# mikostrzewa/AprilSLAM

Hardware: AMD Instinct MI355X
Metric: frames/sec at 1280x720, 20 tags/frame (detection + batched PnP) (higher is better)
Workload: dtype u8/f64

## Files before the change

### aprilslam_amd/csrc/aprilslam.hip

```cpp
#include "../../include/aprilslam.h"

#include <algorithm>
#include <chrono>
#include <cmath>
#include <cstdarg>
#include <cstdio>
#include <cstring>
#include <memory>
#include <string>
#include <type_traits>
#include <vector>

#include "asl_common.h"
#include "tag_standard41h12.inc"
#include "k_wave.inc"

#include "k_threshold.inc"
#include "k_cc.inc"
#include "k_cluster.inc"
#include "k_seg.inc"
#include "k_quad.inc"
#include "k_decode.inc"
#include "k_pnp.inc"
#include "k_dedup.inc"
// ... 231 lines not shown

extern "C" int asl_detector_set_pnp_both_minima(asl_detector *d, int enabled)
{
    if (!d) return fail(ASL_EINVAL, "detector is NULL");
    d->pnp_both_minima = enabled ? 1 : 0;
    return ASL_OK;
}

extern "C" int asl_set_profiling(asl_detector *d, int enabled)
{
    if (!d) return fail(ASL_EINVAL, "detector is NULL");
    d->profiling = enabled ? 1 : 0;
    if (enabled)
        for (int i = 0; i <= MAX_STAGES; i++)
            if (!d->ev[i]) HIPCHK(hipEventCreate(&d->ev[i]));
    return ASL_OK;
}

extern "C" int asl_stage_times(asl_detector *d, const char **names, float *ms, int max_n, int *n)
{
    if (!d || !n) return fail(ASL_EINVAL, "NULL argument");
    int k = std::min(max_n, d->nstages);
    for (int i = 0; i < k; i++) { if (names) names[i] = d->stage_names[i]; if (ms) ms[i] = d->stage_ms[i]; }
    static const char *hn[4] = {"host_enqueue", "host_wait", "host_copy", "host_post"};
    for (int i = 0; i < 4 && k < max_n; i++, k++) { if (names) names[k] = hn[i]; if (ms) ms[k] = d->host_ms[i]; }
    *n = k;
    return ASL_OK;
}

static int pnp_tpw(size_t expected)
{
    const char *e = getenv("ASL_PNP_TPW");
    if (e) { int x = atoi(e); return x < 1 ? 1 : (x > 16 ? 16 : x); }
    int v = 1;
    while (v < 16 && (size_t)v * 2 * 1024 <= expected) v <<= 1;
    return v;
}

static unsigned int next_pow2(unsigned long long v)
{
    unsigned long long p = 1;
    while (p < v) p <<= 1;
    return (unsigned int)p;
}

static int make_geom(asl_detector *d, int n_frames, int channels, int w, int h, int stride, size_t frame_pitch, Geom *g)
{
    if (n_frames <= 0 || n_frames > 65535) return fail(ASL_EINVAL, "n_frames must be in [1, 65535] (got %d)", n_frames);
    if (channels != 1 && channels != 3) return fail(ASL_EINVAL, "channels must be 1 (gray) or 3 (BGR), got %d", channels);
    if (w < 8 || h < 8 || w > 16384 || h > 16384) return fail(ASL_EINVAL, "unsupported image size %dx%d", w, h);
    if (stride < w * channels) return fail(ASL_EINVAL, "stride %d smaller than a row (%d bytes)", stride, w * channels);
    g->w = w; g->h = h; g->stride = stride; g->channels = channels; g->f = d->decimate;
    g->sw = 1 + (w - 1) / g->f; g->sh = 1 + (h - 1) / g->f;
    g->tw = g->sw / TILESZ; g->th = g->sh / TILESZ;
    g->nframes = n_frames; g->frame_pitch = frame_pitch;
    g->npix = (size_t)g->sw * g->sh;
    if (g->npix >= (1u << 24)) return fail(ASL_EINVAL, "decimated frame has %zu pixels; the cluster key holds 2^24", g->npix);
    return ASL_OK;
}

static int seg_nwx(const Geom &g) { return (g.sw + 63) / 64; }
static int seg_point_tiles_y(const Geom &g) { return std::max(1, (g.sh - 1 + SEG_PH - 1) / SEG_PH); }
static size_t count_tiles(const Geom &g) { return (size_t)seg_nwx(g) * (size_t)seg_point_tiles_y(g); }

static int ensure_workspace(asl_detector *d, const Geom &g)
{
    size_t B = (size_t)g.nframes;
    size_t total = B * g.npix;
    d->nslots = next_pow2(std::max<unsigned long long>(16384ull, (unsigned long long)B * d->hash_slots_per_frame));
    unsigned long long mc = (unsigned long long)B * d->clusters_per_frame;
    d->max_clusters = (unsigned int)std::min<unsigned long long>(mc, 0x7FFFFFFFull);
    unsigned long long mp = (unsigned long long)((double)total * d->points_per_pixel) + 65536ull;
    d->max_points = (unsigned int)std::min<unsigned long long>(mp, 0xFFFFFFF0ull);
    d->max_dets = (unsigned int)std::min<unsigned long long>((unsigned long long)B * d->dets_per_frame, 0x7FFFFFFFull);
    int bad = 0;
    bad |= d->dgray.ensure(total);
    bad |= d->tmin.ensure(B * (size_t)std::max(1, g.tw * g.th) + 8);
    bad |= d->tmax.ensure(B * (size_t)std::max(1, g.tw * g.th) + 8);
    bad |= d->tcut.ensure(B * (size_t)std::max(1, g.tw * g.th));
    bad |= d->parent.ensure(total);
    bad |= d->sizes.ensure(total);
    bad |= d->rootmask.ensure(B * (size_t)g.sh * (size_t)seg_nwx(g));
    bad |= d->wmask.ensure(B * (size_t)g.sh * (size_t)seg_nwx(g));
    bad |= d->bmask.ensure(B * (size_t)g.sh * (size_t)seg_nwx(g));
    bad |= d->hkeys.ensure(d->nslots);
    bad |= d->hcounts.ensure(d->nslots);
    bad |= d->class_lists.ensure((size_t)NCLASSES * d->max_clusters);
    bad |= d->slot_cluster.ensure(d->nslots);
    bad |= d->clusters.ensure(d->max_clusters);
    bad |= d->quads.ensure(d->max_clusters);
    bad |= d->quad_list.ensure(d->max_clusters);
    bad |= d->quadH.ensure((size_t)10 * d->max_clusters);
    bad |= d->side_mom.ensure((size_t)24 * d->max_clusters);
    bad |= d->points.ensure(d->max_points);
    d->stage_cap = (unsigned int)((double)g.npix * d->points_per_pixel) + 1024u;
    bad |= d->stage_rec.ensure((size_t)B * d->stage_cap);
    bad |= d->stage_pos.ensure((size_t)B * d->stage_cap);
    bad |= d->frame_cursor.ensure(B);
    bad |= d->dense_tiles.ensure(B * count_tiles(g));
    bad |= d->dense_seg.ensure(B * (size_t)seg_nwx(g) * (size_t)((g.sh + SEG_TH - 1) / SEG_TH));
    bad |= d->seg_edges.ensure(B * (size_t)seg_nwx(g) * (size_t)((g.sh + SEG_TH - 1) / SEG_TH));
    bad |= d->scratch.ensure((size_t)d->max_points * 8);
    bad |= d->dets.ensure(d->max_dets);
    bad |= d->frame_ndets.ensure(B);
    bad |= d->frame_nkeep.ensure(B);
    bad |= d->frame_off.ensure(B);
    bad |= d->frame_idx.ensure(B * (size_t)d->dets_per_frame);
    bad |= d->out_det.ensure(d->max_dets);
    bad |= d->out_pose.ensure(d->max_dets);
    bad |= d->counters.ensure(CNT__N);
    if (bad) return fail(ASL_ENOMEM, "device workspace allocation failed (%zu frames of %dx%d)", B, g.sw, g.sh);
    return ASL_OK;
}

#define STAGE(name)                                                        \
    do {                                                                   \
        if (d->profiling && d->nev < MAX_STAGES) {                         \
            d->stage_names[d->nev] = name;                                 \
            HIPCHK(hipEventRecord(d->ev[d->nev], st));                     \
            d->nev++;                                                      \
        }                                                                  \
    } while (0)

static int tag_width(const asl_detector *d, const Geom &g) { return std::max(3, d->fam.width_at_border / g.f); }

template <int BLOCK, int CAP>
static void launch_fit(asl_detector *d, const Geom &g, int cls, unsigned int grid, hipStream_t st)
{
    const int want_rev = d->fam.reversed_border ? 1 : 0, want_norm = d->fam.reversed_border ? 0 : 1;
    hipLaunchKernelGGL((k_fit_quads<BLOCK, (CAP > 0), CAP / BLOCK>), dim3(grid), dim3(BLOCK), CAP > 0 ? QUAD_LDS_BYTES(CAP) : 0, st, d->clusters.p,
                       d->class_lists.p + (size_t)cls * d->max_clusters, d->counters.p, cls, d->max_clusters, CAP, d->points.p, d->dgray.p, g,
                       tag_width(d, g), want_rev, want_norm, d->scratch.p, d->quads.p, d->wtab.p, d->side_mom.p);
}

static void launch_fit_class(asl_detector *d, const Geom &g, int cls, unsigned int B, hipStream_t st)
{
    const unsigned int qgrid = std::min<unsigned int>(d->max_clusters, std::max<unsigned int>(16384u, 32u * B));
    const unsigned int q2grid = std::min<unsigned int>(d->max_clusters, 2048u);
    switch (cls) {
    case 0: return launch_fit<64, CLASS0_CAP>(d, g, 0, qgrid, st);
    case 1: return launch_fit<128, CLASS1_CAP>(d, g, 1, qgrid, st);
    case 2: return launch_fit<256, CLASS2_CAP>(d, g, 2, q2grid, st);
    case 3: return launch_fit<256, CLASS3_CAP>(d, g, 3, q2grid, st);
    default: return launch_fit<256, 0>(d, g, 4, q2grid, st);
    }
}

static void launch_quad_finish(asl_detector *d, const Geom &g, hipStream_t st)
{
    hipLaunchKernelGGL(k_quad_finish, dim3(std::min<unsigned int>((d->max_clusters + 63) / 64, 4096u)), dim3(256), 0, st, d->quads.p, d->side_mom.p, d->counters.p,
                       d->max_clusters, tag_width(d, g));
}

static int enqueue_detect(asl_detector *d, const uint8_t *d_frames, const Geom &g, hipStream_t st, const CamDev *cam)
{
    dim3 blk(64, 4, 1);
    int thx = (g.sh + TILESZ - 1) / TILESZ;
    unsigned int B = (unsigned int)g.nframes;
    d->nev = 0;
    range_push("S0-S4 gray, decimate, threshold, segmentation, clusters");
    STAGE("k_hash_clear");
    hipLaunchKernelGGL(k_hash_clear, dim3((std::max<unsigned int>(d->nslots, std::max<unsigned int>(B, CNT__N)) + 255) / 256), dim3(256), 0, st, d->hkeys.p,
                       d->hcounts.p, d->nslots, d->counters.p, d->frame_cursor.p, d->frame_ndets.p, B);

    STAGE("k_decimate_minmax");
    if (g.f == 2) {
        const unsigned int ntile = (unsigned int)(g.tw * g.th);
        const unsigned int nrest = (unsigned int)(g.sw - 4 * g.tw) * (unsigned int)g.sh + (unsigned int)(g.sh - 4 * g.th) * (unsigned int)(4 * g.tw);
        if (ntile)
            hipLaunchKernelGGL((g.channels == 1 ? k_decimate2_tiles<1> : k_decimate2_tiles<3>), dim3((ntile + 255) / 256, B), dim3(256), 0, st, d_frames, g,
                               d->dgray.p, d->tmin.p, d->tmax.p);
        if (nrest)
            hipLaunchKernelGGL((g.channels == 1 ? k_decimate_rest<1> : k_decimate_rest<3>), dim3((nrest + 255) / 256, B), dim3(256), 0, st, d_frames, g,
                               d->dgray.p);
    } else
        hipLaunchKernelGGL((g.channels == 1 ? k_decimate_minmax<1> : k_decimate_minmax<3>), dim3((g.sw + 63) / 64, (thx + 3) / 4, B), blk, 0, st, d_frames, g, d->dgray.p, d->tmin.p, d->tmax.p);

    const int nwx = seg_nwx(g), pty = seg_point_tiles_y(g);
    const size_t nwords = (size_t)B * g.sh * nwx;
    STAGE("k_tile_cut");
    if (g.tw > 0 && g.th > 0)
        hipLaunchKernelGGL(k_tile_cut, dim3((((g.tw + 3) / 4) * ((g.th + 3) / 4) + 255) / 256, B), dim3(256), 0, st, d->tmin.p, d->tmax.p, g, d->tcut.p);
    STAGE("k_seg_tile");
    {
        const int ntiles = nwx * ((g.sh + SEG_TH - 1) / SEG_TH);
        hipLaunchKernelGGL(k_seg_tile, dim3((ntiles + SEG_TILE_WAVES - 1) / SEG_TILE_WAVES, 1, B), dim3(64 * SEG_TILE_WAVES), 0, st, d->dgray.p, d->tcut.p, g, nwx, ntiles,
                           d->wmask.p, d->bmask.p, d->parent.p, d->sizes.p, d->rootmask.p, d->seg_edges.p, d->dense_seg.p, d->counters.p);
        hipLaunchKernelGGL(k_seg_tile_dense, dim3(1024), dim3(64), 0, st, g, nwx, ntiles, d->wmask.p, d->bmask.p, d->parent.p, d->sizes.p,
                           d->rootmask.p, d->dense_seg.p, d->counters.p);
    }
    STAGE("k_seg_border");
    {
        const size_t nseams = nwx > 1 ? (size_t)B * g.sh * (nwx - 1) : 0;
        const unsigned int ncol_blocks = (unsigned int)((nseams + 63) / 64);
        const int nrb = (g.sh - 1) / SEG_TH;
        const unsigned int nrow_blocks = (unsigned int)nwx * (unsigned int)nrb * (unsigned int)B;
        if (ncol_blocks + nrow_blocks > 0)
            hipLaunchKernelGGL(k_seg_border, dim3(ncol_blocks + nrow_blocks), dim3(64), 0, st, d->wmask.p, d->bmask.p, d->seg_edges.p,
                               nwx * ((g.sh + SEG_TH - 1) / SEG_TH), g, nwx, d->parent.p, d->counters.p, ncol_blocks, nrb > 0 ? nrb : 1);
    }
    STAGE("k_seg_roots");
    hipLaunchKernelGGL(k_seg_roots, dim3((unsigned int)((nwords + 255) / 256)), dim3(256), 0, st, d->rootmask.p, g, nwx, d->parent.p, d->sizes.p);

    STAGE("k_seg_points");
    hipLaunchKernelGGL((k_seg_points<SEGP_PCAP, SEGP_RUNCAP, SEGP_NW, 1>), dim3(B, (nwx + SEGP_NW - 1) / SEGP_NW, pty), dim3(64 * SEGP_NW), 0, st,
                       d->wmask.p, d->bmask.p, g, nwx, d->parent.p, d->sizes.p, d->hkeys.p, d->hcounts.p, d->nslots - 1, d->stage_rec.p,
                       d->stage_pos.p, d->frame_cursor.p, d->stage_cap, d->dense_tiles.p, pty, d->counters.p);
    hipLaunchKernelGGL((k_seg_points<SEGP_PCAP_DENSE, SEGP_RUNCAP_DENSE, 1, 2>), dim3(256), dim3(64), 0, st, d->wmask.p, d->bmask.p, g, nwx,
                       d->parent.p, d->sizes.p, d->hkeys.p, d->hcounts.p, d->nslots - 1, d->stage_rec.p, d->stage_pos.p, d->frame_cursor.p,
                       d->stage_cap, d->dense_tiles.p, pty, d->counters.p);
    STAGE("k_cluster_filter");
    hipLaunchKernelGGL(k_cluster_filter, dim3((d->nslots + 1023) / 1024), dim3(1024), 0, st, d->hkeys.p, d->hcounts.p, d->nslots, g,
                       d->clusters.p, d->slot_cluster.p, d->class_lists.p, d->max_clusters, d->max_points, d->counters.p);
    STAGE("k_point_place");
    hipLaunchKernelGGL(k_point_place, dim3(16, B), dim3(256), 0, st, d->stage_rec.p, d->stage_pos.p, d->frame_cursor.p, d->stage_cap,
                       d->slot_cluster.p, d->points.p, d->counters.p);

    range_pop();
    range_push("S5 quad fit");
    for (int cls = 0; cls < NCLASSES; cls++) {
        static const char *const kFitStage[NCLASSES] = {"k_fit_quads<0>", "k_fit_quads<1>", "k_fit_quads<2>", "k_fit_quads<3>", "k_fit_quads<4>"};
        STAGE(kFitStage[cls]);
        launch_fit_class(d, g, cls, B, st);
    }

    STAGE("k_quad_finish");
    launch_quad_finish(d, g, st);
    range_pop();
    range_push("S6-S7 edge refinement, homography, decode");
    STAGE("k_quad_compact");
    hipLaunchKernelGGL(k_quad_compact, dim3((d->max_clusters + 1023) / 1024), dim3(1024), 0, st, d->quads.p, d->counters.p, d->max_clusters,
                       d->quad_list.p);
    unsigned int dgrid = std::min<unsigned int>(d->max_clusters, std::max<unsigned int>(8192u, 64u * B));
    STAGE("k_refine");
    hipLaunchKernelGGL((g.channels == 1 ? k_refine<1> : k_refine<3>), dim3(dgrid), dim3(64), 0, st, d->quads.p, d->counters.p, d->max_clusters, d_frames, g,
                       d->fam.reversed_border ? 1 : 0, d->refine, d->quadH.p, d->quad_list.p, d->side_mom.p);
    STAGE("k_homography");
    hipLaunchKernelGGL(k_homography, dim3(std::min<unsigned int>((d->max_clusters + 31) / 32, 2048u)), dim3(256), 0, st, d->quadH.p, d->counters.p, d->max_clusters,
                       d->quad_list.p, d->side_mom.p);
    STAGE("k_decode");
    hipLaunchKernelGGL((g.channels == 1 ? k_decode<1> : k_decode<3>), dim3(dgrid), dim3(64), 0, st, d->quads.p, d->quadH.p, d->counters.p, d->max_clusters, d_frames, g, d->fam,
                       d->maxhamming, d->dets.p, d->max_dets, d->counters.p, d->quad_list.p);

    range_pop();
    range_push("S9 PnP, S8 de-duplication");
    if (cam) {
        STAGE("k_pnp_dets");
        const int tpw = pnp_tpw(d->nd_guess ? d->nd_guess : (size_t)20 * B);
        hipLaunchKernelGGL(k_pnp_dets, dim3((d->max_dets + tpw - 1) / tpw), dim3(64), 0, st, d->dets.p, d->counters.p, d->max_dets, *cam, tpw);
    }
    STAGE("k_det_dedup");
    {
        const unsigned int cap_f = d->dets_per_frame;
        hipLaunchKernelGGL(k_det_bucket, dim3((d->max_dets + 255) / 256), dim3(256), 0, st, d->dets.p, d->counters.p, d->max_dets, d->frame_ndets.p,
                           d->frame_idx.p, cap_f, d->counters.p);
        hipLaunchKernelGGL(k_det_dedup, dim3(B), dim3(256), 0, st, d->dets.p, d->counters.p, d->frame_ndets.p, d->frame_idx.p, cap_f,
                           d->frame_nkeep.p, d->counters.p);
        hipLaunchKernelGGL(k_det_offsets, dim3(1), dim3(1024), 0, st, d->frame_nkeep.p, B, d->frame_off.p, d->counters.p);
        hipLaunchKernelGGL(k_det_gather, dim3((cap_f + 255) / 256, B), dim3(256), 0, st, d->dets.p, d->frame_idx.p, cap_f, d->frame_nkeep.p,
                           d->frame_off.p, d->out_det.p, d->out_pose.p, d->max_dets, cam ? 1 : 0);
    }
    range_pop();
    if (d->profiling && d->nev <= MAX_STAGES) HIPCHK(hipEventRecord(d->ev[d->nev], st));
    HIPCHK(hipGetLastError());
    return ASL_OK;
}

static CamDev make_cam(const asl_detector *d, const double *K, const double *dist, int n_dist, double tag_size)
{
    CamDev c;
    c.both_minima = d->pnp_both_minima; c.pad = 0;
    c.fx = K[0]; c.fy = K[4]; c.cx = K[2]; c.cy = K[5];
    c.k1 = c.k2 = c.p1 = c.p2 = c.k3 = 0;
    if (dist && n_dist >= 4) { c.k1 = dist[0]; c.k2 = dist[1]; c.p1 = dist[2]; c.p2 = dist[3]; }
    if (dist && n_dist >= 5) c.k3 = dist[4];
    c.half = (double)(float)(tag_size / 2);
    return c;
}

using clk = std::chrono::steady_clock;
static float msf(clk::time_point a, clk::time_point b) { return std::chrono::duration<float, std::milli>(b - a).count(); }

static int ensure_host_out(asl_detector *d, size_t want, size_t nframes)
{
    HIPCHK(d->host_nkeep.ensure(nframes, hipHostMallocDefault));
    if (want <= d->host_cap()) return ASL_OK;
    d->host_det.release(); d->host_pose.release();
    want = std::max<size_t>(want * 2, 4096);
    HIPCHK(d->host_det.ensure(want, hipHostMallocNonCoherent));
    HIPCHK(d->host_pose.ensure(want, hipHostMallocNonCoherent));
    return ASL_OK;
}

static int submit_batch(asl_detector *d, const uint8_t *d_frames, const Geom &g, hipStream_t st, const CamDev *cam)
{
    if (d->pending) return fail(ASL_EINVAL, "a batch is already in flight on this detector: collect it first");
    int rc = ensure_workspace(d, g);
    if (rc) return rc;
    d->t_submit = clk::now();
    rc = enqueue_detect(d, d_frames, g, st, cam);
    if (rc) return rc;
    HIPCHK(d->pinned_counters.ensure(CNT__N, hipHostMallocDefault));
    HIPCHK(hipMemcpyAsync(d->pinned_counters.p, d->counters.p, sizeof(long long) * CNT__N, hipMemcpyDeviceToHost, st));
    d->prefetched = 0;
    rc = ensure_host_out(d, std::min<size_t>(d->nd_guess, d->max_dets), (size_t)g.nframes);
    if (rc) return rc;
    HIPCHK(hipMemcpyAsync(d->host_nkeep.p, d->frame_nkeep.p, sizeof(unsigned int) * (size_t)g.nframes, hipMemcpyDeviceToHost, st));
    if (d->nd_guess > 0) {
        size_t guess = std::min<size_t>(d->nd_guess, d->max_dets);
        HIPCHK(hipMemcpyAsync(d->host_det.p, d->out_det.p, guess * sizeof(DetOut), hipMemcpyDeviceToHost, st));
        if (cam) HIPCHK(hipMemcpyAsync(d->host_pose.p, d->out_pose.p, guess * sizeof(PoseOut), hipMemcpyDeviceToHost, st));
        d->prefetched = guess;
    }
    d->pending = true;
    d->p_frames = d_frames; d->p_geom = g; d->p_stream = st; d->p_has_cam = cam != nullptr;
    if (cam) d->p_cam = *cam;
    d->t_enqueued = clk::now();
    return ASL_OK;
}

static int collect_batch(asl_detector *d, asl_detection *out, asl_pose *poses, int max_out, int *n_per_frame, int *n_out)
{
    if (!d->pending) return fail(ASL_EINVAL, "no batch in flight on this detector");
    const Geom g = d->p_geom;
    hipStream_t st = d->p_stream;
    const CamDev *cam = d->p_has_cam ? &d->p_cam : nullptr;
    clk::time_point t0 = d->t_submit, t1 = d->t_enqueued, t2 = t1;
    for (int attempt = 0; attempt < 4; attempt++) {
        if (attempt > 0) {
            d->pending = false;
            d->nd_guess = 0;
            int rc = submit_batch(d, d->p_frames, g, st, cam);
            if (rc) return rc;
        }
        HIPCHK(hipStreamSynchronize(st));
        t2 = clk::now();
        memcpy(d->last_counters, d->pinned_counters.p, sizeof(long long) * CNT__N);
        d->last = g;
        long long *c = d->last_counters;
        if (c[CNT_UF_GUARD]) {
            d->pending = false;
            return fail(ASL_ECAPACITY, "a union-find loop hit its iteration guard (%lld times): labels of this batch are not trustworthy", c[CNT_UF_GUARD]);
        }
        bool again = false;
        if (c[CNT_OVERFLOW_HASH]) { d->hash_slots_per_frame *= 4; again = true; }
        if (c[CNT_OVERFLOW_CLUSTERS] || c[CNT_NCLUSTERS] > (long long)d->max_clusters) { d->clusters_per_frame *= 4; again = true; }
        if (c[CNT_OVERFLOW_POINTS]) { d->points_per_pixel *= 2; again = true; }
        if (c[CNT_OVERFLOW_DETS]) { d->dets_per_frame *= 4; again = true; }
        if (again) {
            if (attempt == 3) {
                d->pending = false;
                return fail(ASL_ECAPACITY, "work buffers still overflow after growing (hash %lld clusters %lld points %lld dets %lld)",
                            c[CNT_OVERFLOW_HASH], c[CNT_OVERFLOW_CLUSTERS], c[CNT_OVERFLOW_POINTS], c[CNT_OVERFLOW_DETS]);
            }
            continue;
        }
        break;
    }
    d->pending = false;
    if (d->profiling) {
        d->nstages = d->nev;
        for (int i = 0; i < d->nev; i++) HIPCHK(hipEventElapsedTime(&d->stage_ms[i], d->ev[i], d->ev[i + 1]));
    }
    if (d->last_counters[CNT_DEDUP_LIMIT])
        return fail(ASL_ECAPACITY, "%lld frame(s) hold more than %d detections: the de-duplication does not sort that many", d->last_counters[CNT_DEDUP_LIMIT], DEDUP_MAX);
    size_t nd = (size_t)d->last_counters[CNT_NKEEP];
    if (nd > d->max_dets) nd = d->max_dets;
    if (nd > d->prefetched) {
        size_t have = d->prefetched;
        if (nd > d->host_cap()) have = 0;
        int rc = ensure_host_out(d, nd, (size_t)g.nframes);
        if (rc) return rc;
        HIPCHK(hipMemcpy(d->host_det.p + have, d->out_det.p + have, (nd - have) * sizeof(DetOut), hipMemcpyDeviceToHost));
        if (cam) HIPCHK(hipMemcpy(d->host_pose.p + have, d->out_pose.p + have, (nd - have) * sizeof(PoseOut), hipMemcpyDeviceToHost));
    }
    d->nd_guess = nd + nd / 4 + 256;
    clk::time_point t3 = clk::now();
    static_assert(sizeof(DetOut) == sizeof(asl_detection) && sizeof(PoseOut) == sizeof(asl_pose), "device results are copied verbatim");
    int total = (int)nd;
    int nw = std::min(total, max_out);
    if (out && nw > 0) memcpy(out, d->host_det.p, (size_t)nw * sizeof(asl_detection));
    if (poses && cam && nw > 0) memcpy(poses, d->host_pose.p, (size_t)nw * sizeof(asl_pose));
    if (n_per_frame) for (int f = 0; f < g.nframes; f++) n_per_frame[f] = (int)d->host_nkeep.p[f];
    if (n_out) *n_out = total;
    d->host_ms[0] = msf(t0, t1); d->host_ms[1] = msf(t1, t2); d->host_ms[2] = msf(t2, t3); d->host_ms[3] = msf(t3, clk::now());
    return ASL_OK;
}

// ... 810 lines not shown
```

### aprilslam_amd/csrc/k_decode.inc

```

#define DEC_PROBE_GROUP 11
#define DEC_MAX_PROBES 44

__device__ __forceinline__ void half_angle_normal_dev(double a, double b, double *nx, double *ny)
{
    double r = sqrt(a * a + b * b);
    if (r == 0) { *nx = 1; *ny = 0; return; }
    double c2 = a / r;
    if (c2 >= 0) {
        double c = sqrt((1 + c2) / 2);
        *nx = c;
        *ny = b / (2 * r * c);
    } else {
        double s = sqrt((1 - c2) / 2);
        if (b < 0) s = -s;
        *ny = s;
        *nx = b / (2 * r * s);
    }
}

__device__ __forceinline__ double grp8_max(double v)
{
    v = fmax(v, dpp_mov<QUAD_XOR1>(0.0, v));
    v = fmax(v, dpp_mov<QUAD_XOR2>(0.0, v));
    return fmax(v, dpp_mov<0x141>(0.0, v));
}
__device__ __forceinline__ int grp8_min(int v)
{
    v = min(v, dpp_mov<QUAD_XOR1>(0, v));
    v = min(v, dpp_mov<QUAD_XOR2>(0, v));
    return min(v, dpp_mov<0x141>(0, v));
}
__device__ __forceinline__ int grp8_owner(bool mine, int lane)
{
    const unsigned long long m = __ballot(mine);
    return (lane & ~7) + (__ffs((int)((m >> (lane & ~7)) & 0xFFull)) - 1);
}

__global__ void __launch_bounds__(256) k_homography(double *__restrict__ corners_H, const long long *__restrict__ counters, unsigned int max_clusters,
                                                    const unsigned int *__restrict__ quad_list, const double *__restrict__ edge_mom)
{
    if (batch_poisoned(counters)) return;
    const long long nq64 = counters[CNT_NQUADS];
    const unsigned int nq = nq64 > (long long)max_clusters ? max_clusters : (unsigned int)nq64;
    const int lane = threadIdx.x & 63, r = lane & 7;
    for (unsigned int q0 = blockIdx.x * 32u; q0 < nq; q0 += gridDim.x * 32u) {
        const unsigned int qi = q0 + (threadIdx.x >> 3);
        const bool live = qi < nq;
        const unsigned int ci = quad_list[live ? qi : 0];
        double *const rec = corners_H + 10 * (size_t)ci;
        const double state = live ? rec[9] : 0.0;
        const bool todo = state == 0.5 || state == 0.25;
        const int e = r & 3;
        double Pex = todo ? rec[2 * e] : 0.0, Pey = todo ? rec[2 * e + 1] : 0.0;
        if (__any(state == 0.25)) {
            const double *in = edge_mom + ((size_t)(state == 0.25 ? ci : 0) * 4 + e) * 6;
            const double Mx = in[0], My = in[1], Mxx = in[2], Mxy = in[3], Myy = in[4], Nn = in[5];
            const double Ex = Mx / Nn, Ey = My / Nn;
            const double Cxx = Mxx / Nn - Ex * Ex, Cxy = Mxy / Nn - Ex * Ey, Cyy = Myy / Nn - Ey * Ey;
            double nx, ny;
            half_angle_normal_dev(Cyy - Cxx, -2 * Cxy, &nx, &ny);
            const double n0 = dpp_mov<QUAD_ROT1>(0.0, Ex), n1 = dpp_mov<QUAD_ROT1>(0.0, Ey), n2 = dpp_mov<QUAD_ROT1>(0.0, nx), n3 = dpp_mov<QUAD_ROT1>(0.0, ny);
            const double A00 = ny, A01 = -n3;
            const double A10 = -nx, A11 = n2;
            const double B0 = -Ex + n0;
            const double B1 = -Ey + n1;
            const double det = A00 * A11 - A10 * A01;
            const bool moved = fabs(det) > 0.001;
            const double W00 = A11 / det, W01 = -A01 / det;
            const double L0 = W00 * B0 + W01 * B1;
            const double cx = Ex + L0 * A00, cy = Ey + L0 * A10;
            const double fx = dpp_mov<QUAD_ROT3>(0.0, cx), fy = dpp_mov<QUAD_ROT3>(0.0, cy);
            const bool fm = dpp_mov<QUAD_ROT3>(0, moved ? 1 : 0) != 0;
            if (state == 0.25 && fm) { Pex = fx; Pey = fy; }
        }
        const int i = r >> 1;
        const double x = (i == 1 || i == 2) ? 1.0 : -1.0, y = (i >= 2) ? 1.0 : -1.0;
        const double u = __shfl(Pex, (lane & ~7) + i), v = __shfl(Pey, (lane & ~7) + i);
        double a[9];
        if ((r & 1) == 0) { a[0] = x; a[1] = y; a[2] = 1; a[3] = 0; a[4] = 0; a[5] = 0; a[6] = -x * u; a[7] = -y * u; a[8] = u; }
        else { a[0] = 0; a[1] = 0; a[2] = 0; a[3] = x; a[4] = y; a[5] = 1; a[6] = -x * v; a[7] = -y * v; a[8] = v; }
        int pos = r;
        bool ok = true;
#pragma unroll
        for (int col = 0; col < 8; col++) {
            const double val = pos >= col ? fabs(a[col]) : -1.0;
            const double mx = grp8_max(val);
            if (mx < 1e-10) ok = false;
            const int pivpos = grp8_min(val == mx ? pos : 99);
            const bool is_piv = pos == pivpos;
            if (is_piv) pos = col;
            else if (pos == col) pos = pivpos;
            const int src = grp8_owner(is_piv, lane);
            double piv[9];
#pragma unroll
            for (int j = col; j < 9; j++) piv[j] = __shfl(a[j], src);
            if (pos > col) {
                const double f = a[col] / piv[col];
                a[col] = 0.0;
#pragma unroll
                for (int j = col + 1; j < 9; j++) a[j] = a[j] - f * piv[j];
            }
        }
        double xs[8], mine = 0;
#pragma unroll
        for (int col = 7; col >= 0; col--) {
            double sum = 0;
#pragma unroll
            for (int k = col + 1; k < 8; k++) sum += a[k] * xs[k];
            const double xc = (a[8] - sum) / a[col];
            xs[col] = __shfl(xc, grp8_owner(pos == col, lane));
            if (r == col) mine = xs[col];
        }
        const bool all_ok = (__ballot(ok) >> (lane & ~7) & 0xFFull) == 0xFFull;
        if (todo) {
            rec[r] = mine;
            if (r == 0) { rec[8] = 1.0; rec[9] = all_ok ? 1.0 : 0.0; }
        }
    }
}

__device__ __forceinline__ void hproject_dev(const double *H, double x, double y, double *ox, double *oy)
{
    double xx = H[0] * x + H[1] * y + H[2];
    double yy = H[3] * x + H[4] * y + H[5];
    double zz = H[6] * x + H[7] * y + H[8];
    *ox = xx / zz;
    *oy = yy / zz;
}

struct GrayModel { double A[9], B[3], C[3]; };

__device__ __forceinline__ void gm_add_dev(GrayModel &gm, double x, double y, double gray)
{
    gm.A[0] += x * x; gm.A[1] += x * y; gm.A[2] += x; gm.A[4] += y * y; gm.A[5] += y; gm.A[8] += 1;
    gm.B[0] += x * gray; gm.B[1] += y * gray; gm.B[2] += gray;
}

__device__ __forceinline__ void gm_solve_dev(GrayModel &gm)
{
    const double *A = gm.A, *B = gm.B;
    double L[9], M[9], t[3];
    L[0] = sqrt(A[0]); L[3] = A[1] / L[0]; L[6] = A[2] / L[0];
    L[4] = sqrt(A[4] - L[3] * L[3]); L[7] = (A[5] - L[3] * L[6]) / L[4];
    L[8] = sqrt(A[8] - L[6] * L[6] - L[7] * L[7]);
    M[0] = 1 / L[0]; M[3] = -L[3] * M[0] / L[4]; M[4] = 1 / L[4];
    M[6] = (-L[6] * M[0] - L[7] * M[3]) / L[8]; M[7] = -L[7] * M[4] / L[8]; M[8] = 1 / L[8];
    t[0] = M[0] * B[0]; t[1] = M[3] * B[0] + M[4] * B[1]; t[2] = M[6] * B[0] + M[7] * B[1] + M[8] * B[2];
    gm.C[0] = M[0] * t[0] + M[3] * t[1] + M[6] * t[2];
    gm.C[1] = M[4] * t[1] + M[7] * t[2];
    gm.C[2] = M[8] * t[2];
}

__device__ __forceinline__ double gm_interp_dev(const GrayModel &gm, double x, double y) { return gm.C[0] * x + gm.C[1] * y + gm.C[2]; }

template <int CH>
__device__ __forceinline__ double value_for_pixel_dev(const uint8_t *frame, const Geom &g, double px, double py)
{
    int x1 = (int)floor(px - 0.5), x2 = (int)ceil(px - 0.5);
    double x = px - 0.5 - x1;
    int y1 = (int)floor(py - 0.5), y2 = (int)ceil(py - 0.5);
    double y = py - 0.5 - y1;
    if (x1 < 0 || x2 >= g.w || y1 < 0 || y2 >= g.h) return -1;
    return gray_at<CH>(frame, g, x1, y1) * (1 - x) * (1 - y) + gray_at<CH>(frame, g, x2, y1) * x * (1 - y) +
           gray_at<CH>(frame, g, x1, y2) * (1 - x) * y + gray_at<CH>(frame, g, x2, y2) * x * y;
}

__device__ __forceinline__ unsigned long long rotate90_dev(unsigned long long w, int nbits)
{
    int p = nbits;
    unsigned long long l = 0;
    if (nbits % 4 == 1) { p = nbits - 1; l = 1; }
    w = ((w >> l) << (p / 4 + l)) | (w >> (3 * p / 4 + l) << l) | (w & l);
    w &= ((1ull << nbits) - 1ull);
    return w;
}

#define PIX_EPS 9.5367431640625e-07

template <int CH>
__global__ void __launch_bounds__(64) k_refine(const QuadRec *__restrict__ quads, const long long *__restrict__ counters,
                                               unsigned int max_clusters, const uint8_t *__restrict__ frames, Geom g, int fam_reversed,
                                               int refine, double *__restrict__ Hout ,
                                               const unsigned int *__restrict__ quad_list, double *__restrict__ edge_mom )
{
    __shared__ double s_bx[64], s_by[64];
    __shared__ int s_bvalid[64];
    __shared__ double s_P[4][2];
    __shared__ int s_soff[5];
    __shared__ short s_probe[DEC_MAX_PROBES][64];
    __shared__ double s_enx[4], s_eny[4];
    int lane = threadIdx.x;
    PHASE_DECL();
    if (batch_poisoned(counters)) return;
    long long nq64 = counters[CNT_NQUADS];
    unsigned int nq = nq64 > (long long)max_clusters ? max_clusters : (unsigned int)nq64;

    for (unsigned int qi = blockIdx.x; qi < nq; qi += gridDim.x) {
        __syncthreads();
        PHASE_INIT();
        const unsigned int ci = quad_list[qi];
        const QuadRec *qp = quads + ci;
        const int q_valid = qp->valid, q_reversed = qp->reversed_border;
        if (lane == 0) Hout[10 * (size_t)ci + 9] = 0.0;
        if (!q_valid) continue;
        if (fam_reversed != q_reversed) continue;
        int fr = (int)(qp->key >> 48);
        const uint8_t *frame = frames + (size_t)fr * g.frame_pitch;
        if (lane < 4) {
            double px = qp->p[lane][0], py = qp->p[lane][1];
            if (g.f > 1) { px = (px - 0.5) * g.f + 0.5; py = (py - 0.5) * g.f + 0.5; }
            s_P[lane][0] = px;
            s_P[lane][1] = py;
        }
        __syncthreads();

        PHASE(16);
        if (refine) {
            if (lane < 4) {
                int edge = lane, a = edge, b = (edge + 1) & 3;
                double nx = s_P[b][1] - s_P[a][1], ny = -s_P[b][0] + s_P[a][0];
                double mag = sqrt(nx * nx + ny * ny);
                nx /= mag; ny /= mag;
                if (q_reversed) { nx = -nx; ny = -ny; }
                int ns = (int)(mag / 8);
                if (ns < 16) ns = 16;
                s_enx[edge] = nx; s_eny[edge] = ny;
                int n0 = __shfl(ns, 0), n1 = __shfl(ns, 1), n2 = __shfl(ns, 2), n3 = __shfl(ns, 3);
                if (lane == 0) { s_soff[0] = 0; s_soff[1] = n0; s_soff[2] = n0 + n1; s_soff[3] = n0 + n1 + n2; s_soff[4] = n0 + n1 + n2 + n3; }
            }
            __syncthreads();
            PHASE(24);
            const int *soff = s_soff;
            const double *enx = s_enx, *eny = s_eny;
            const double range = g.f + 1;
            const int steps = (int)(2 * range * 4) + 1;
            const int nprobe = steps + 8;
            double Mx = 0, My = 0, Mxx = 0, Mxy = 0, Myy = 0, Nn = 0;
            const int total = soff[4];
            for (int base = 0; base < total; base += 64) {
            {
                const int idx = base + lane;
                if (idx < total) {
                int edge = idx >= soff[3] ? 3 : (idx >= soff[2] ? 2 : (idx >= soff[1] ? 1 : 0));
                int sidx = idx - soff[edge];
                int a = edge, b = (edge + 1) & 3;
                double pax = s_P[a][0], pay = s_P[a][1], pbx = s_P[b][0], pby = s_P[b][1];
                double nx = enx[edge], ny = eny[edge];
                int nsamples = soff[edge + 1] - soff[edge];
                double alpha = (1.0 + sidx) / (nsamples + 1);
                double x0 = alpha * pax + (1 - alpha) * pbx;
                double y0 = alpha * pay + (1 - alpha) * pby;
                double Mn = 0, Mcount = 0;
                if (nprobe <= DEC_MAX_PROBES) {
                    const double t_first = -(range + 1), t_last = -(range + 1) + 0.25 * (nprobe - 1);
                    const int xa = (int)(x0 + t_first * nx + PIX_EPS), xb = (int)(x0 + t_last * nx + PIX_EPS);
                    const int ya = (int)(y0 + t_first * ny + PIX_EPS), yb = (int)(y0 + t_last * ny + PIX_EPS);
                    const bool clear = min(xa, xb) >= 0 && max(xa, xb) <= g.w - 2 && min(ya, yb) >= 0 && max(ya, yb) <= g.h - 1;
                    if (__all(clear)) {
                        unsigned int at_prev = 0xFFFFFFFFu;
                        int gray_prev = 0;
                        for (int j0 = 0; j0 < nprobe; j0 += DEC_PROBE_GROUP) {
                            const double tb = -(range + 1) + 0.25 * j0;
                            unsigned int raw[DEC_PROBE_GROUP], at[DEC_PROBE_GROUP];
#pragma unroll
                            for (int u = 0; u < DEC_PROBE_GROUP; u++) {
                                const double t = tb + 0.25 * u;
                                const int xi = (int)(x0 + t * nx + PIX_EPS), yi = (int)(y0 + t * ny + PIX_EPS);
                                at[u] = j0 + u < nprobe ? (unsigned int)yi * (unsigned int)g.stride + (unsigned int)(CH * xi) : 0xFFFFFFFEu;
                            }
#pragma unroll
                            for (int u = 0; u < DEC_PROBE_GROUP; u++) {
                                raw[u] = 0;
                                if (j0 + u < nprobe && at[u] != (u ? at[u - 1] : at_prev)) {
                                    if (CH == 1) raw[u] = frame[at[u]];
                                    else __builtin_memcpy(&raw[u], frame + at[u], 4);
                                }
                            }
#pragma unroll
                            for (int u = 0; u < DEC_PROBE_GROUP; u++) {
                                if (j0 + u < nprobe) {
                                    const bool fresh = at[u] != (u ? at[u - 1] : at_prev);
                                    gray_prev = fresh ? (CH == 1 ? (int)raw[u] : bgr_gray(raw[u])) : gray_prev;
                                    s_probe[j0 + u][lane] = (short)gray_prev;
                                }
                            }
                            at_prev = at[DEC_PROBE_GROUP - 1];
                        }
                    } else
                    for (int j0 = 0; j0 < nprobe; j0 += DEC_PROBE_GROUP) {
                        unsigned int raw[DEC_PROBE_GROUP], shv[DEC_PROBE_GROUP];
                        bool inside[DEC_PROBE_GROUP];
#pragma unroll
                        for (int u = 0; u < DEC_PROBE_GROUP; u++) {
                            double t = -(range + 1) + 0.25 * (j0 + u);
                            int xi = (int)(x0 + t * nx + PIX_EPS), yi = (int)(y0 + t * ny + PIX_EPS);
                            inside[u] = j0 + u < nprobe && (unsigned int)xi < (unsigned int)g.w && (unsigned int)yi < (unsigned int)g.h;
                            raw[u] = pixel_fetch<CH>(frame, g, inside[u] ? xi : 0, inside[u] ? yi : 0, &shv[u]);
                        }
#pragma unroll
                        for (int u = 0; u < DEC_PROBE_GROUP; u++)
                            if (j0 + u < nprobe) s_probe[j0 + u][lane] = inside[u] ? (short)pixel_gray<CH>(raw[u], shv[u]) : (short)-1;
                    }
                    PHASE(25);
                    int isum = 0, wsum = 0;
                    const int k0 = 4 * (g.f + 1);
                    for (int k = 0; k < steps; k++) {
                        const int g1 = s_probe[k + 8][lane], g2 = s_probe[k][lane];
                        const int dg = g2 - g1;
                        const int wgt = (g1 < 0 || g2 < 0 || g1 < g2) ? 0 : dg * dg;
                        isum += wgt * (k - k0);
                        wsum += wgt;
                    }
                    Mn = 0.25 * (double)isum;
                    Mcount = (double)wsum;
                } else {
                    for (int k = 0; k < steps; k++) {
                        double n = -range + 0.25 * k;
                        int x1 = (int)(x0 + (n + 1) * nx + PIX_EPS), y1 = (int)(y0 + (n + 1) * ny + PIX_EPS);
                        if (x1 < 0 || x1 >= g.w || y1 < 0 || y1 >= g.h) continue;
                        int x2 = (int)(x0 + (n - 1) * nx + PIX_EPS), y2 = (int)(y0 + (n - 1) * ny + PIX_EPS);
                        if (x2 < 0 || x2 >= g.w || y2 < 0 || y2 >= g.h) continue;
                        int g1 = gray_at<CH>(frame, g, x1, y1), g2 = gray_at<CH>(frame, g, x2, y2);
                        if (g1 < g2) continue;
                        double weight = (double)((g2 - g1) * (g2 - g1));
                        Mn += weight * n;
                        Mcount += weight;
                    }
                }
                if (Mcount == 0) { s_bvalid[lane] = 0; }
                else {
                    double n0 = Mn / Mcount;
                    s_bx[lane] = x0 + n0 * nx;
                    s_by[lane] = y0 + n0 * ny;
                    s_bvalid[lane] = 1;
                }
                }
            }
            __syncthreads();
            PHASE(26);
            if (lane < 4) {
                const int edge = lane;
                const int lo = (soff[edge] > base ? soff[edge] : base) - base;
                const int hi = (soff[edge + 1] < base + 64 ? soff[edge + 1] : base + 64) - base;
                for (int k = lo; k < hi; k++) {
                    if (!s_bvalid[k]) continue;
                    double bx = s_bx[k], by = s_by[k];
                    Mx += bx; My += by; Mxx += bx * bx; Mxy += bx * by; Myy += by * by; Nn++;
                }
            }
            __syncthreads();
            PHASE(27);
            }
            if (lane < 4) {
                double *out = edge_mom + ((size_t)ci * 4 + lane) * 6;
                out[0] = Mx; out[1] = My; out[2] = Mxx; out[3] = Mxy; out[4] = Myy; out[5] = Nn;
            }
        }

        PHASE(17);
        if (lane < 8) Hout[10 * (size_t)ci + lane] = s_P[lane >> 1][lane & 1];
        if (lane == 0) Hout[10 * (size_t)ci + 9] = refine ? 0.25 : 0.5;
        PHASE(22);
    }
    PHASE_FLUSH(16);
}

template <int CH>
__global__ void __launch_bounds__(64) __attribute__((amdgpu_waves_per_eu(5))) k_decode(const QuadRec *__restrict__ quads, const double *__restrict__ Hin,
                                               const long long *__restrict__ counters, unsigned int max_clusters,
                                               const uint8_t *__restrict__ frames, Geom g, FamilyDev fam, int maxhamming, DetRec *dets,
                                               unsigned int max_dets, long long *wcounters, const unsigned int *__restrict__ quad_list)
{
    __shared__ double s_H[9];
    __shared__ double s_smp[40][4];
    __shared__ double s_values[16 * 16], s_list[2 * 64];
    __shared__ double s_smpxy[40][2], s_bitxy[64][2];
    __shared__ GrayModel s_white, s_black;
    __shared__ int s_ok;
    int lane = threadIdx.x;
    PHASE_DECL();
    if (batch_poisoned(counters)) return;
    long long nq64 = counters[CNT_NQUADS];
    unsigned int nq = nq64 > (long long)max_clusters ? max_clusters : (unsigned int)nq64;

    {
        const int wb = fam.width_at_border;
        if (lane < 8 * wb && lane < 40) {
            int pi = lane / wb, i = lane % wb;
            double p0, p1, p2, p3;
            switch (pi) {
            case 0: p0 = -0.5; p1 = 0.5; p2 = 0; p3 = 1; break;
            case 1: p0 = 0.5; p1 = 0.5; p2 = 0; p3 = 1; break;
            case 2: p0 = wb + 0.5; p1 = .5; p2 = 0; p3 = 1; break;
            case 3: p0 = wb - 0.5; p1 = .5; p2 = 0; p3 = 1; break;
            case 4: p0 = 0.5; p1 = -0.5; p2 = 1; p3 = 0; break;
            case 5: p0 = 0.5; p1 = 0.5; p2 = 1; p3 = 0; break;
            case 6: p0 = 0.5; p1 = wb + 0.5; p2 = 1; p3 = 0; break;
            default: p0 = 0.5; p1 = wb - 0.5; p2 = 1; p3 = 0; break;
            }
            double tagx01 = (p0 + i * p2) / wb, tagy01 = (p1 + i * p3) / wb;
            s_smpxy[lane][0] = 2 * (tagx01 - 0.5);
            s_smpxy[lane][1] = 2 * (tagy01 - 0.5);
        }
        if (lane < fam.nbits) {
            int bitx = fam.bit_x[lane], bity = fam.bit_y[lane];
            double tagx01 = (bitx + 0.5) / wb, tagy01 = (bity + 0.5) / wb;
            s_bitxy[lane][0] = 2 * (tagx01 - 0.5);
            s_bitxy[lane][1] = 2 * (tagy01 - 0.5);
        }
    }
    for (unsigned int qi = blockIdx.x; qi < nq; qi += gridDim.x) {
        __syncthreads();
        PHASE_INIT();
        const unsigned int ci = quad_list[qi];
        if (Hin[10 * (size_t)ci + 9] == 0.0) continue;
        unsigned long long qkey = quads[ci].key;
        int fr = (int)(qkey >> 48);
        const uint8_t *frame = frames + (size_t)fr * g.frame_pitch;
        if (lane < 9) s_H[lane] = Hin[10 * (size_t)ci + lane];
        __syncthreads();
        int wb = fam.width_at_border, tw = fam.total_width;

        PHASE(18);
        int nsmp = 8 * wb;
        if (lane < nsmp && lane < 40) {
            const double tagx = s_smpxy[lane][0], tagy = s_smpxy[lane][1];
            double px, py;
            hproject_dev(s_H, tagx, tagy, &px, &py);
            int ix = (int)px, iy = (int)py;
            const bool inside = !(ix < 0 || iy < 0 || ix >= g.w || iy >= g.h);
            const double gv = (double)gray_at<CH>(frame, g, inside ? ix : 0, inside ? iy : 0);
            s_smp[lane][0] = inside ? tagx : 0.0; s_smp[lane][1] = inside ? tagy : 0.0; s_smp[lane][2] = inside ? gv : 0.0; s_smp[lane][3] = inside ? 1.0 : 0.0;
        }
        __syncthreads();
        {
            const int a = lane % 9, m = lane / 9;
            const int ku = a <= 2 ? 0 : (a <= 4 ? 1 : (a == 5 ? 3 : (a == 6 ? 0 : (a == 7 ? 1 : 2))));
            const int kv = a == 0 ? 0 : (a == 1 ? 1 : (a == 3 ? 1 : (a == 6 || a == 7 ? 2 : 3)));
            double acc = 0;
            if (lane < 18) {
                const int ns = nsmp < 40 ? nsmp : 40;
                for (int p0 = m * wb; p0 < ns; p0 += 2 * wb) {
                    const int pe = p0 + wb < ns ? p0 + wb : ns;
                    for (int smp = p0; smp < pe; smp++) {
                        const double u = s_smp[smp][ku], v = s_smp[smp][kv];
                        acc += u * v;
                    }
                }
            }
            GrayModel gm;
            const int base = (lane & 1) * 9;
            gm.A[0] = __shfl(acc, base + 0); gm.A[1] = __shfl(acc, base + 1); gm.A[2] = __shfl(acc, base + 2);
            gm.A[3] = 0; gm.A[4] = __shfl(acc, base + 3); gm.A[5] = __shfl(acc, base + 4);
            gm.A[6] = 0; gm.A[7] = 0; gm.A[8] = __shfl(acc, base + 5);
            gm.B[0] = __shfl(acc, base + 6); gm.B[1] = __shfl(acc, base + 7); gm.B[2] = __shfl(acc, base + 8);
            gm.C[0] = 0; gm.C[1] = 0; gm.C[2] = 0;
            gm_solve_dev(gm);
            if (lane == 0) s_white = gm;
            if (lane == 1) s_black = gm;
            const double at0 = gm_interp_dev(gm, 0, 0);
            const double w0 = __shfl(at0, 0), b0 = __shfl(at0, 1);
            if (lane == 0) {
                bool flip = (w0 - b0 < 0);
                s_ok = (flip == (fam.reversed_border != 0)) ? 1 : 0;
            }
        }
        for (int i = lane; i < tw * tw; i += 64) s_values[i] = 0;
        __syncthreads();
        if (!s_ok) continue;

        PHASE(19);
        int min_coord = (wb - tw) / 2;
        int bit_cell = 0, cell_x = 0, cell_y = 0;
        if (lane < fam.nbits) {
            int bitx = fam.bit_x[lane], bity = fam.bit_y[lane];
            cell_x = bitx - min_coord; cell_y = bity - min_coord;
            bit_cell = tw * cell_y + cell_x;
            const double tagx = s_bitxy[lane][0], tagy = s_bitxy[lane][1];
            double px, py;
            hproject_dev(s_H, tagx, tagy, &px, &py);
            double v = value_for_pixel_dev<CH>(frame, g, px, py);
            if (v != -1) {
                double thresh = (gm_interp_dev(s_black, tagx, tagy) + gm_interp_dev(s_white, tagx, tagy)) / 2.0;
                s_values[bit_cell] = v - thresh;
            }
        }
        __syncthreads();
        double sharp_v = 0.0;
        if (lane < fam.nbits) {
            double sv = 0;
            if (cell_y - 1 >= 0) sv += s_values[bit_cell - tw] * -1.0;
            if (cell_x - 1 >= 0) sv += s_values[bit_cell - 1] * -1.0;
            sv += s_values[bit_cell] * 4.0;
            if (cell_x + 1 <= tw - 1) sv += s_values[bit_cell + 1] * -1.0;
            if (cell_y + 1 <= tw - 1) sv += s_values[bit_cell + tw] * -1.0;
            sharp_v = s_values[bit_cell] + 0.25 * sv;
        }

        PHASE(20);
        float black_score, white_score, black_count, white_count;
        unsigned long long rcode;
        {
            const bool isbit = lane < fam.nbits;
            const double v = isbit ? sharp_v : 0.0;
            const bool isw = isbit && v > 0;
            const unsigned long long wm = __ballot(isw), bm = __ballot(isbit && !isw);
            rcode = __brevll(wm) >> (64 - fam.nbits);
            const unsigned long long below = (1ull << lane) - 1ull;
            if (isbit) s_list[isw ? __popcll(wm & below) : 64 + __popcll(bm & below)] = isw ? v : -v;
// ... 84 lines not shown
```

Before: 377,800.

## Specialize edge refine on decimation factor with register-packed probes and dot2 sums

Templates k_refine on the decimation factor so probe counts are compile-time, and keeps the probe grays packed four per 32-bit register instead of a shared-memory probe array. The weighted step sums use packed u16 saturating subtract with udot2. The per-edge moment reduction moves from 4 serial lanes to 24 lanes, one per moment, using a shared moment table and a ballot valid mask. It also sets a waves-per-EU occupancy hint. These aim to cut LDS traffic and serial reduction latency, at the cost of more kernel instantiations and register pressure.

Result: faster. 384,000 (median of 6 runs) (+1.6%).

```diff
diff --git a/aprilslam_amd/csrc/aprilslam.hip b/aprilslam_amd/csrc/aprilslam.hip
--- a/aprilslam_amd/csrc/aprilslam.hip
+++ b/aprilslam_amd/csrc/aprilslam.hip
@@ -407,6 +407,18 @@
                        d->max_clusters, tag_width(d, g));
 }
 
+template <int CH>
+static auto refine_kernel_ch(int f) -> decltype(&k_refine<CH, 0>)
+{
+    switch (f) {
+    case 1: return k_refine<CH, 1>;
+    case 2: return k_refine<CH, 2>;
+    case 3: return k_refine<CH, 3>;
+    default: return k_refine<CH, 0>;
+    }
+}
+static auto refine_kernel(const Geom &g) -> decltype(&k_refine<1, 0>) { return g.channels == 1 ? refine_kernel_ch<1>(g.f) : refine_kernel_ch<3>(g.f); }
+
 static int enqueue_detect(asl_detector *d, const uint8_t *d_frames, const Geom &g, hipStream_t st, const CamDev *cam)
 {
     dim3 blk(64, 4, 1);
@@ -488,7 +500,7 @@
                        d->quad_list.p);
     unsigned int dgrid = std::min<unsigned int>(d->max_clusters, std::max<unsigned int>(8192u, 64u * B));
     STAGE("k_refine");
-    hipLaunchKernelGGL((g.channels == 1 ? k_refine<1> : k_refine<3>), dim3(dgrid), dim3(64), 0, st, d->quads.p, d->counters.p, d->max_clusters, d_frames, g,
+    hipLaunchKernelGGL(refine_kernel(g), dim3(dgrid), dim3(64), 0, st, d->quads.p, d->counters.p, d->max_clusters, d_frames, g,
                        d->fam.reversed_border ? 1 : 0, d->refine, d->quadH.p, d->quad_list.p, d->side_mom.p);
     STAGE("k_homography");
     hipLaunchKernelGGL(k_homography, dim3(std::min<unsigned int>((d->max_clusters + 31) / 32, 2048u)), dim3(256), 0, st, d->quadH.p, d->counters.p, d->max_clusters,
diff --git a/aprilslam_amd/csrc/k_decode.inc b/aprilslam_amd/csrc/k_decode.inc
--- a/aprilslam_amd/csrc/k_decode.inc
+++ b/aprilslam_amd/csrc/k_decode.inc
@@ -1,6 +1,7 @@
 
+#ifndef DEC_PROBE_GROUP
 #define DEC_PROBE_GROUP 11
-#define DEC_MAX_PROBES 44
+#endif
 
 __device__ __forceinline__ void half_angle_normal_dev(double a, double b, double *nx, double *ny)
 {
@@ -178,23 +179,141 @@
 
 #define PIX_EPS 9.5367431640625e-07
 
-template <int CH>
-__global__ void __launch_bounds__(64) k_refine(const QuadRec *__restrict__ quads, const long long *__restrict__ counters,
+template <int F>
+struct RefineDims {
+    static constexpr int STEPS = 8 * (F + 1) + 1;
+    static constexpr int NPROBE = STEPS + 8;
+    static constexpr int ND = (NPROBE + 3) / 4;
+};
+
+typedef unsigned short refine_u16x2 __attribute__((ext_vector_type(2)));
+
+#define REFINE_GROUP_FENCE(x0, y0, nx, ny) asm volatile("" : "+v"(x0), "+v"(y0), "+v"(nx), "+v"(ny) : : "memory")
+
+template <int CH, int F>
+__device__ __forceinline__ void refine_probes_clear(const uint8_t *__restrict__ frame, unsigned int stride, double x0, double y0, double nx, double ny,
+                                                    unsigned int (&P)[RefineDims<F>::ND])
+{
+    constexpr int NPROBE = RefineDims<F>::NPROBE;
+    unsigned int at_prev = 0xFFFFFFFFu;
+    int gray_prev = 0;
+#pragma unroll
+    for (int j0 = 0; j0 < NPROBE; j0 += DEC_PROBE_GROUP) {
+        REFINE_GROUP_FENCE(x0, y0, nx, ny);
+        unsigned int raw[DEC_PROBE_GROUP], at[DEC_PROBE_GROUP];
+#pragma unroll
+        for (int u = 0; u < DEC_PROBE_GROUP; u++) {
+            if (j0 + u >= NPROBE) continue;
+            const double t = -(double)(F + 2) + 0.25 * (j0 + u);
+            const int xi = (int)(x0 + t * nx + PIX_EPS), yi = (int)(y0 + t * ny + PIX_EPS);
+            at[u] = (unsigned int)yi * stride + (unsigned int)(CH * xi);
+        }
+#pragma unroll
+        for (int u = 0; u < DEC_PROBE_GROUP; u++) {
+            if (j0 + u >= NPROBE) continue;
+            raw[u] = 0;
+            if (at[u] != (u ? at[u - 1] : at_prev)) {
+                if (CH == 1) raw[u] = frame[at[u]];
+                else __builtin_memcpy(&raw[u], frame + at[u], 4);
+            }
+        }
+#pragma unroll
+        for (int u = 0; u < DEC_PROBE_GROUP; u++) {
+            const int j = j0 + u;
+            if (j >= NPROBE) continue;
+            const bool fresh = at[u] != (u ? at[u - 1] : at_prev);
+            gray_prev = fresh ? (CH == 1 ? (int)raw[u] : bgr_gray(raw[u])) : gray_prev;
+            if ((j & 3) == 0) P[j >> 2] = (unsigned int)gray_prev;
+            else P[j >> 2] |= (unsigned int)gray_prev << (8 * (j & 3));
+        }
+        if (j0 + DEC_PROBE_GROUP < NPROBE) at_prev = at[DEC_PROBE_GROUP - 1];
+    }
+}
+
+template <int CH, int F>
+__device__ __forceinline__ unsigned long long refine_probes_checked(const uint8_t *__restrict__ frame, const Geom &g, double x0, double y0, double nx,
+                                                                    double ny, unsigned int (&P)[RefineDims<F>::ND])
+{
+    constexpr int NPROBE = RefineDims<F>::NPROBE;
+    unsigned long long inside_mask = 0;
+#pragma unroll
+    for (int d = 0; d < RefineDims<F>::ND; d++) {
+        REFINE_GROUP_FENCE(x0, y0, nx, ny);
+        unsigned int raw[4], shv[4], in4 = 0;
+#pragma unroll
+        for (int u = 0; u < 4; u++) {
+            const int j = 4 * d + u;
+            if (j >= NPROBE) continue;
+            const double t = -(double)(F + 2) + 0.25 * j;
+            const int xi = (int)(x0 + t * nx + PIX_EPS), yi = (int)(y0 + t * ny + PIX_EPS);
+            const bool inside = (unsigned int)xi < (unsigned int)g.w && (unsigned int)yi < (unsigned int)g.h;
+            raw[u] = pixel_fetch<CH>(frame, g, inside ? xi : 0, inside ? yi : 0, &shv[u]);
+            in4 |= inside ? 1u << u : 0u;
+        }
+        unsigned int p = 0;
+#pragma unroll
+        for (int u = 0; u < 4; u++)
+            if (4 * d + u < NPROBE) p |= (unsigned int)pixel_gray<CH>(raw[u], shv[u]) << (8 * u);
+        P[d] = p;
+        inside_mask |= (unsigned long long)in4 << (4 * d);
+    }
+    return inside_mask;
+}
+
+template <int F, bool MASKED>
+__device__ __forceinline__ void refine_step_sums(const unsigned int (&P)[RefineDims<F>::ND], unsigned long long inside_mask, unsigned int *ksum,
+                                                 unsigned int *wsum)
+{
+    constexpr int STEPS = RefineDims<F>::STEPS;
+    const unsigned long long both = inside_mask & (inside_mask >> 8);
+    unsigned int ks = 0, ws = 0;
+#pragma unroll
+    for (int d = 0; 4 * d < STEPS; d++) {
+#pragma unroll
+        for (int h = 0; h < 2; h++) {
+            const int ka = 4 * d + h, kb = ka + 2;
+            if (ka >= STEPS) continue;
+            const unsigned int lo = P[d], hi = P[d + 2];
+            const refine_u16x2 g2 = __builtin_bit_cast(refine_u16x2, h ? __builtin_amdgcn_perm(0u, lo, 0x0c030c01u) : lo & 0x00FF00FFu);
+            const refine_u16x2 g1 = __builtin_bit_cast(refine_u16x2, h ? __builtin_amdgcn_perm(0u, hi, 0x0c030c01u) : hi & 0x00FF00FFu);
+            const refine_u16x2 dg = __builtin_elementwise_sub_sat(g1, g2);
+            refine_u16x2 wgt = dg * dg;
+            if (MASKED) {
+                const unsigned int m = ((both >> ka & 1ull) ? 0x0000FFFFu : 0u) | ((both >> kb & 1ull) ? 0xFFFF0000u : 0u);
+                wgt = __builtin_bit_cast(refine_u16x2, __builtin_bit_cast(unsigned int, wgt) & m);
+            }
+            const bool two = kb < STEPS;
+            const refine_u16x2 ones = {1, (unsigned short)(two ? 1 : 0)}, kk = {(unsigned short)ka, (unsigned short)(two ? kb : 0)};
+            ws = __builtin_amdgcn_udot2(wgt, ones, ws, false);
+            ks = __builtin_amdgcn_udot2(wgt, kk, ks, false);
+        }
+    }
+    *ksum = ks;
+    *wsum = ws;
+}
+
+#define REFINE_MOM(k, e, m) (6 * (k) + 6 * (e) + (m))
+#define REFINE_MOM_SIZE (6 * 64 + 6 * 3)
+
+#ifndef DEC_REFINE_WAVES
+#define DEC_REFINE_WAVES 5
+#endif
+template <int CH, int F>
+__global__ void __launch_bounds__(64) __attribute__((amdgpu_waves_per_eu(DEC_REFINE_WAVES))) k_refine(const QuadRec *__restrict__ quads, const long long *__restrict__ counters,
                                                unsigned int max_clusters, const uint8_t *__restrict__ frames, Geom g, int fam_reversed,
                                                int refine, double *__restrict__ Hout ,
                                                const unsigned int *__restrict__ quad_list, double *__restrict__ edge_mom )
 {
-    __shared__ double s_bx[64], s_by[64];
-    __shared__ int s_bvalid[64];
+    __shared__ __attribute__((aligned(16))) double s_mom[REFINE_MOM_SIZE];
     __shared__ double s_P[4][2];
     __shared__ int s_soff[5];
-    __shared__ short s_probe[DEC_MAX_PROBES][64];
     __shared__ double s_enx[4], s_eny[4];
     int lane = threadIdx.x;
     PHASE_DECL();
     if (batch_poisoned(counters)) return;
     long long nq64 = counters[CNT_NQUADS];
     unsigned int nq = nq64 > (long long)max_clusters ? max_clusters : (unsigned int)nq64;
+    const int f = F ? F : g.f;
 
     for (unsigned int qi = blockIdx.x; qi < nq; qi += gridDim.x) {
         __syncthreads();
@@ -209,7 +328,7 @@
         const uint8_t *frame = frames + (size_t)fr * g.frame_pitch;
         if (lane < 4) {
             double px = qp->p[lane][0], py = qp->p[lane][1];
-            if (g.f > 1) { px = (px - 0.5) * g.f + 0.5; py = (py - 0.5) * g.f + 0.5; }
+            if (f > 1) { px = (px - 0.5) * f + 0.5; py = (py - 0.5) * f + 0.5; }
             s_P[lane][0] = px;
             s_P[lane][1] = py;
         }
@@ -233,12 +352,11 @@
             PHASE(24);
             const int *soff = s_soff;
             const double *enx = s_enx, *eny = s_eny;
-            const double range = g.f + 1;
-            const int steps = (int)(2 * range * 4) + 1;
-            const int nprobe = steps + 8;
-            double Mx = 0, My = 0, Mxx = 0, Mxy = 0, Myy = 0, Nn = 0;
+            const int acc_edge = lane / 6, acc_m = lane - 6 * acc_edge;
+            double acc = 0;
             const int total = soff[4];
             for (int base = 0; base < total; base += 64) {
+            bool bvalid = false;
             {
                 const int idx = base + lane;
                 if (idx < total) {
@@ -252,69 +370,29 @@
                 double x0 = alpha * pax + (1 - alpha) * pbx;
                 double y0 = alpha * pay + (1 - alpha) * pby;
                 double Mn = 0, Mcount = 0;
-                if (nprobe <= DEC_MAX_PROBES) {
-                    const double t_first = -(range + 1), t_last = -(range + 1) + 0.25 * (nprobe - 1);
+                if (F != 0) {
+                    constexpr int FF = F ? F : 1;
+                    unsigned int P[RefineDims<FF>::ND];
+                    unsigned int ksum, wsum;
+                    const double t_first = -(double)(FF + 2), t_last = -(double)(FF + 2) + 0.25 * (RefineDims<FF>::NPROBE - 1);
                     const int xa = (int)(x0 + t_first * nx + PIX_EPS), xb = (int)(x0 + t_last * nx + PIX_EPS);
                     const int ya = (int)(y0 + t_first * ny + PIX_EPS), yb = (int)(y0 + t_last * ny + PIX_EPS);
                     const bool clear = min(xa, xb) >= 0 && max(xa, xb) <= g.w - 2 && min(ya, yb) >= 0 && max(ya, yb) <= g.h - 1;
                     if (__all(clear)) {
-                        unsigned int at_prev = 0xFFFFFFFFu;
-                        int gray_prev = 0;
-                        for (int j0 = 0; j0 < nprobe; j0 += DEC_PROBE_GROUP) {
-                            const double tb = -(range + 1) + 0.25 * j0;
-                            unsigned int raw[DEC_PROBE_GROUP], at[DEC_PROBE_GROUP];
-#pragma unroll
-                            for (int u = 0; u < DEC_PROBE_GROUP; u++) {
-                                const double t = tb + 0.25 * u;
-                                const int xi = (int)(x0 + t * nx + PIX_EPS), yi = (int)(y0 + t * ny + PIX_EPS);
-                                at[u] = j0 + u < nprobe ? (unsigned int)yi * (unsigned int)g.stride + (unsigned int)(CH * xi) : 0xFFFFFFFEu;
-                            }
-#pragma unroll
-                            for (int u = 0; u < DEC_PROBE_GROUP; u++) {
-                                raw[u] = 0;
-                                if (j0 + u < nprobe && at[u] != (u ? at[u - 1] : at_prev)) {
-                                    if (CH == 1) raw[u] = frame[at[u]];
-                                    else __builtin_memcpy(&raw[u], frame + at[u], 4);
-                                }
-                            }
-#pragma unroll
-                            for (int u = 0; u < DEC_PROBE_GROUP; u++) {
-                                if (j0 + u < nprobe) {
-                                    const bool fresh = at[u] != (u ? at[u - 1] : at_prev);
-                                    gray_prev = fresh ? (CH == 1 ? (int)raw[u] : bgr_gray(raw[u])) : gray_prev;
-                                    s_probe[j0 + u][lane] = (short)gray_prev;
-                                }
-                            }
-                            at_prev = at[DEC_PROBE_GROUP - 1];
-                        }
-                    } else
-                    for (int j0 = 0; j0 < nprobe; j0 += DEC_PROBE_GROUP) {
-                        unsigned int raw[DEC_PROBE_GROUP], shv[DEC_PROBE_GROUP];
-                        bool inside[DEC_PROBE_GROUP];
-#pragma unroll
-                        for (int u = 0; u < DEC_PROBE_GROUP; u++) {
-                            double t = -(range + 1) + 0.25 * (j0 + u);
-                            int xi = (int)(x0 + t * nx + PIX_EPS), yi = (int)(y0 + t * ny + PIX_EPS);
-                            inside[u] = j0 + u < nprobe && (unsigned int)xi < (unsigned int)g.w && (unsigned int)yi < (unsigned int)g.h;
-                            raw[u] = pixel_fetch<CH>(frame, g, inside[u] ? xi : 0, inside[u] ? yi : 0, &shv[u]);
-                        }
-#pragma unroll
-                        for (int u = 0; u < DEC_PROBE_GROUP; u++)
-                            if (j0 + u < nprobe) s_probe[j0 + u][lane] = inside[u] ? (short)pixel_gray<CH>(raw[u], shv[u]) : (short)-1;
+                        refine_probes_clear<CH, FF>(frame, (unsigned int)g.stride, x0, y0, nx, ny, P);
+                        PHASE(25);
+                        refine_step_sums<FF, false>(P, 0ull, &ksum, &wsum);
+                    } else {
+                        const unsigned long long inside_mask = refine_probes_checked<CH, FF>(frame, g, x0, y0, nx, ny, P);
+                        PHASE(25);
+                        refine_step_sums<FF, true>(P, inside_mask, &ksum, &wsum);
                     }
-                    PHASE(25);
-                    int isum = 0, wsum = 0;
-                    const int k0 = 4 * (g.f + 1);
-                    for (int k = 0; k < steps; k++) {
-                        const int g1 = s_probe[k + 8][lane], g2 = s_probe[k][lane];
-                        const int dg = g2 - g1;
-                        const int wgt = (g1 < 0 || g2 < 0 || g1 < g2) ? 0 : dg * dg;
-                        isum += wgt * (k - k0);
-                        wsum += wgt;
-                    }
+                    const int isum = (int)ksum - 4 * (FF + 1) * (int)wsum;
                     Mn = 0.25 * (double)isum;
-                    Mcount = (double)wsum;
+                    Mcount = (double)(int)wsum;
                 } else {
+                    const double range = f + 1;
+                    const int steps = (int)(2 * range * 4) + 1;
                     for (int k = 0; k < steps; k++) {
                         double n = -range + 0.25 * k;
                         int x1 = (int)(x0 + (n + 1) * nx + PIX_EPS), y1 = (int)(y0 + (n + 1) * ny + PIX_EPS);
@@ -328,34 +406,28 @@
                         Mcount += weight;
                     }
                 }
-                if (Mcount == 0) { s_bvalid[lane] = 0; }
-                else {
+                if (Mcount != 0) {
                     double n0 = Mn / Mcount;
-                    s_bx[lane] = x0 + n0 * nx;
-                    s_by[lane] = y0 + n0 * ny;
-                    s_bvalid[lane] = 1;
-                }
-                }
-            }
+                    const double bx = x0 + n0 * nx, by = y0 + n0 * ny;
+                    double *row = s_mom + REFINE_MOM(lane, edge, 0);
+                    row[0] = bx; row[1] = by; row[2] = bx * bx; row[3] = bx * by; row[4] = by * by; row[5] = 1.0;
+                    bvalid = true;
+                }
+                }
+            }
+            const unsigned long long valid_mask = __ballot(bvalid);
             __syncthreads();
             PHASE(26);
-            if (lane < 4) {
-                const int edge = lane;
-                const int lo = (soff[edge] > base ? soff[edge] : base) - base;
-                const int hi = (soff[edge + 1] < base + 64 ? soff[edge + 1] : base + 64) - base;
-                for (int k = lo; k < hi; k++) {
-                    if (!s_bvalid[k]) continue;
-                    double bx = s_bx[k], by = s_by[k];
-                    Mx += bx; My += by; Mxx += bx * bx; Mxy += bx * by; Myy += by * by; Nn++;
-                }
+            if (lane < 24) {
+                const int lo = (soff[acc_edge] > base ? soff[acc_edge] : base) - base;
+                const int hi = (soff[acc_edge + 1] < base + 64 ? soff[acc_edge + 1] : base + 64) - base;
+                for (int k = lo; k < hi; k++)
+                    if (valid_mask >> k & 1ull) acc += s_mom[REFINE_MOM(k, acc_edge, acc_m)];
             }
             __syncthreads();
             PHASE(27);
             }
-            if (lane < 4) {
-                double *out = edge_mom + ((size_t)ci * 4 + lane) * 6;
-                out[0] = Mx; out[1] = My; out[2] = Mxx; out[3] = Mxy; out[4] = Myy; out[5] = Nn;
-            }
+            if (lane < 24) edge_mom[(size_t)ci * 24 + lane] = acc;
         }
 
         PHASE(17);
```
